# fan1994song/Sentinel

Measured on AMD Instinct MI355X. Metric: flow-check decisions/sec (node) + % HBM roofline, 10M resources, 1/2/4/8 GPU, higher is better.
Workload: dtype int64; 1 GPU; config3: 10M resources Zipf(1.1), 60% QPS / 10% THREAD / 15% WarmUp / 15% RateLimiter, acquireCount 1 (90%) or 2-5, RT~Exp(20ms) exits; events_per_batch_per_gpu=134217728, entries_per_batch_per_gpu=122837294, parallelism=resource-sharded x1, trace=config-3 batch, seed 3

## Files before the change

### sentinel_amd/csrc/sf_internal.h

```cpp
#pragma once
#include <hip/hip_runtime.h>
#include <stdint.h>

#include "../../include/sentinel_flow.h"
#include "sf_degrade.h"
#include "sf_authority.h"

namespace sf {

constexpr int64_t WS_NONE = -(1LL << 62);
constexpr int MINUTE = SF_MINUTE_BUCKETS;
constexpr int MAX_RULES = SF_MAX_RULES_PER_RESOURCE;

struct Bucket {
    int64_t ws, pass, block, exc, succ, rt, occ, min_rt;
};
struct Borrow {
    int64_t ws, pass;
};

enum : int32_t { CT_DEFAULT = 0, CT_WARM_UP = 1, CT_RATE_LIMITER = 2, CT_WARM_UP_RATE_LIMITER = 3 };

struct DevRule {
    uint8_t kind, grade;
// ... 197 lines not shown
    uint32_t arg_slots; const uint8_t* nargs; const uint8_t* atag; const uint64_t* abits;
    uint32_t arg_stride;
    const uint32_t* aoff; const uint8_t* etag; const uint64_t* ebits;
    uint32_t acsr;
    const uint32_t* origin; const uint32_t* ctx;
    int64_t base;
    const uint8_t* sys;
    const uint8_t* vprev;
    uint8_t marked;
};
struct DevVerdicts { uint8_t* status; int32_t* wait; uint16_t* rule; };

constexpr uint8_t EVF_SYSBLK = 0x80u;
constexpr uint8_t EVF_SYSREASON_SHIFT = 4;
constexpr uint8_t SYS_NONE = 0xFFu;
constexpr uint8_t SYS_INERT = 0xFEu;
constexpr uint8_t SYSR_OTHER = 7;
constexpr uint8_t SYSR_AUTH = 6;
constexpr int64_t EREF_DEAD = -2;

hipError_t query_temp_bytes(uint32_t max_n, size_t* sort_bytes, size_t* scan_bytes, size_t* pscan_bytes);
hipError_t launch_init_state(const DevState& st, hipStream_t s);
hipError_t launch_rdesc(const DevState& st, hipStream_t s);
hipError_t launch_entry_node(const DevState& st, const DevBatch& b, const uint8_t* vstatus, EntryNode* en,
                             EntryAcc* acc, hipStream_t s);
hipError_t launch_entry_init(EntryNode* en, int64_t max_rt, hipStream_t s);
hipError_t rocprim_scan_bytes(uint32_t n, size_t* bytes);
hipError_t launch_en_pack_ws(const EntryNode* en, int S, int64_t* ws, hipStream_t s);
hipError_t launch_en_pack_vals(const EntryNode* en, int S, const int64_t* gws, int64_t* vals, int64_t* minrt,
                               hipStream_t s);
hipError_t launch_snapshot(const DevState& st, int64_t now, uint32_t shard_count, uint32_t shard_index,
                           uint32_t* counts, uint32_t* offsets, sf_metric_row* out, uint32_t cap, uint32_t* total,
                           void* scan_tmp, size_t scan_bytes, hipStream_t s);
hipError_t mlog_temp_bytes(uint32_t nodes, uint32_t rows, size_t* bytes);
hipError_t launch_mlog_count(const DevState& st, EntryNode* en, bool with_entry, uint32_t shard_count,
                             uint32_t shard_index, int64_t now, unsigned long long* mask, uint32_t* counts,
                             uint32_t* offsets, uint32_t* total, void* tmp, size_t tmp_bytes, unsigned grid,
                             hipEvent_t after_count, hipStream_t s);
hipError_t launch_mlog_rows(const DevState& st, EntryNode* en, bool with_entry, uint32_t shard_count,
                            uint32_t shard_index, int64_t now, const unsigned long long* mask, const uint32_t* offsets,
                            uint32_t n_rows, sf_metric_row* rows, uint8_t* keys, uint8_t* keys_out, uint32_t* order,
                            uint32_t* order_out, void* tmp, size_t tmp_bytes, unsigned grid, hipStream_t s);
hipError_t launch_fmt_len(const sf_metric_row* rows, const uint32_t* order, uint32_t n, const char* names,
                          const uint64_t* name_off, const int32_t* types, uint32_t n_names, int64_t tz,
                          uint64_t* line_len, uint64_t* line_off, uint64_t* total, void* tmp, size_t tmp_bytes,
                          hipStream_t s);
hipError_t launch_fmt_write(const sf_metric_row* rows, const uint32_t* order, uint32_t n, const char* names,
                            const uint64_t* name_off, const int32_t* types, uint32_t n_names, int64_t tz,
                            const uint64_t* line_off, char* out, hipStream_t s);
hipError_t launch_param_stats(const DevState& st, unsigned long long* out, hipStream_t s);
size_t segs_lb_bytes(uint32_t max_n);
hipError_t launch_node_digests(const DevState& st, uint32_t n, unsigned long long* out, hipStream_t s);
hipError_t launch_param_thread_read(const DevState& st, uint32_t l, int idx, uint32_t tag, uint64_t bits,
                                    long long* out, hipStream_t s);
hipError_t launch_sort(const DevState& st, Work& w, const DevBatch& b, uint32_t shard_count, uint32_t shard_index,
                       uint32_t key_bits, hipStream_t s, hipEvent_t* ev, bool timing, bool classify = true);
struct OxWin { int64_t w0s, w0m; uint32_t ws, wm; };
struct OxPlan { uint32_t n_heavy, n_pairs; OxWin win; };
hipError_t launch_decide(const DevState& st, Work& w, const DevBatch& b, const DevVerdicts& out,
                         hipStream_t s, hipStream_t s2, hipStream_t s3, hipStream_t s4, hipEvent_t* ev, bool timing,
                         const OxPlan* ox = nullptr, bool classify = false, hipStream_t sv = nullptr);
hipError_t launch_pk_expand(const uint64_t* ev, const uint32_t* ev4, const uint32_t* ms_end, uint32_t n_ms,
                            const int64_t* xref, const int64_t* xcts, const int32_t* cext,
                            int64_t base, uint32_t n, uint32_t n_exit, uint32_t n_cext, uint2* tile_cnt,
                            uint32_t* res, int64_t* ts, int32_t* cnt, uint8_t* flags, int64_t* eref, int64_t* cts,
                            int32_t* err, hipStream_t s);
struct PkArgIn; struct PkArgOut;
struct PkCopy {
    const uint8_t* etag; const uint64_t* ebits; uint8_t* etag_out; uint64_t* ebits_out;
    const uint32_t* ctx; uint32_t* ctx_out; const uint32_t* origin; uint32_t* origin_out;
};
hipError_t launch_pk_args(const PkArgIn& in, const PkArgOut& out, const PkCopy& cp, int32_t* err, hipStream_t s);
hipError_t launch_sparse_verdicts(const int32_t* wait, const uint16_t* rule, uint32_t n, unsigned long long* wl,
                                  unsigned long long* rl, uint32_t* counts, hipStream_t s);
hipError_t launch_auth_mark(const AuthTables& t, const uint32_t* res, const uint32_t* origin, const uint8_t* flags,
                            uint32_t n, uint8_t mark, uint8_t* out, hipStream_t s);
hipError_t launch_ox_index(const DevState& st, Work& w, const DevBatch& b, uint32_t lim, hipStream_t s);
hipError_t launch_ox_apply(const DevState& st, Work& w, const DevBatch& b, uint32_t n_heavy, uint32_t n_pairs,
                           const OxWin& win, hipStream_t s);
hipError_t launch_ox_rehash(const ParamSlot* old_tab, uint64_t old_n, ParamSlot* new_tab, uint64_t new_mask,
                            int32_t* err, hipStream_t s);
hipError_t launch_aux_find(const DevState& st, uint64_t hi, uint64_t lo, uint32_t* out, hipStream_t s);
constexpr size_t ACC_BYTES = 72;
constexpr int SF_NUM_EVENTS = 18;

}
```

### sentinel_amd/csrc/sf_kernels.hip

```cpp
#include <cstring>
#include <rocprim/rocprim.hpp>

#include "sf_pkargs.h"
#include "sf_rsort.h"
#include "sf_stream.h"
#include "sf_system.h"
#include "sf_xflow.h"

namespace sf {

__global__ void k_init_state(DevState st, size_t n_sec, size_t n_min) {
    size_t i = (size_t)blockIdx.x * blockDim.x + threadIdx.x;
    size_t stride = (size_t)gridDim.x * blockDim.x;
    for (size_t k = i; k < n_sec; k += stride) {
        st.second[k] = fresh_bucket(WS_NONE, st.max_rt);
        st.borrow[k].ws = WS_NONE; st.borrow[k].pass = 0;
    }
    for (size_t k = i; k < n_min; k += stride) st.minute[k] = fresh_bucket(WS_NONE, st.max_rt);
    for (size_t k = i; k < st.R; k += stride) st.threads[k] = 0;
}

__global__ void k_segs(DevBatch b, SortedEv ev, const uint8_t* s_atag,
                       const uint32_t* keys, const uint32_t* head_scan, uint32_t* seg_start, uint32_t* seg_res,
                       uint32_t* n_seg, uint32_t* segflag, int64_t* last_ts, const int32_t* err, bool exit_marks,
// ... 1003 lines not shown
                crow.blk = (unsigned long long)v[0]; crow.succ = (unsigned long long)v[1];
                crow.rt = (unsigned long long)v[2]; crow.exc = (unsigned long long)v[3];
                crow.thr = v[4] + (long long)__popcll(__ballot(npss != 0)); crow.pass = (unsigned long long)v[5];
                crow.minrt = mr;
                crow.nblk = (unsigned)__popcll(__ballot(nblk != 0)); crow.ncmp = (unsigned)__popcll(__ballot(ncmp != 0));
                crow.nexc = (unsigned)__popcll(__ballot(nexc != 0)); crow.npass = (unsigned)__popcll(__ballot(npss != 0));
            }
            XW_PF(2)
            if (nblk || ncmp || npss) {
                if (jac) {
                    if (my_row > 0) xw_add(rows[my_row], blk, nblk, succ, rt, minrt, exc, nexc, thr, ncmp, pss, npss);
                } else if (origin != SF_ORIGIN_NONE) {
                    uint32_t h = 1 + (uint32_t)(mix64(origin) % (XW_KCAP - 1));
                    for (;;) {
                        const unsigned int prev = atomicCAS(&rows[h].key, 0u, origin + 1u);
                        if (prev == 0u || prev == origin + 1u) break;
                        h = h + 1 < XW_KCAP ? h + 1 : 1;
                    }
                    xw_add(rows[h], blk, nblk, succ, rt, minrt, exc, nexc, thr, ncmp, pss, npss);
                }
            }
            __syncthreads();
            XW_PF(3)
            if (lane == 0) xw_apply<MAXS>(cn, crow, t0);
            if constexpr (MAXS == 2) {
                if (jac) {
                    for (uint32_t k = 1 + lane; k < XW_KCAP; k += 64)
                        if ((rows[k].nblk | rows[k].ncmp | rows[k].npass | rows[k].nexc) && oc.ko[k - 1] != XNONE)
                            xw_apply<2>(xw_node(ocnw, k - 1), rows[k], t0);
                }
            }
            for (uint32_t k = 1 + lane; k < XW_KCAP && !jac; k += 64) {
                if (!rows[k].key) continue;
                const uint32_t ko = aux_get(st, l, AX_ORIGIN, rows[k].key - 1u);
                if (ko == XNONE) continue;
                NodeWin<MAXS> x;
                const NodeRows nr = aux_rows(st, ko);
                nw_load(x, st, nr);
                xw_apply<MAXS>(x, rows[k], t0);
                nw_store(x, st, nr);
            }
            XW_PF(4)
            if (act) vch[lane] = vfin;
            __syncthreads();
            jprev = j0;
            e = nx;
            XW_PF(5)
            j0 = jn;
        }
#ifdef SF_XW_PROFILE
        if (lane == 0 && hi - lo > 20000)
            printf("xw seg n=%u chunks=%llu setup=%llu solve=%llu (%llu %llu %llu %llu %llu %llu) post %llu %llu %llu %llu %llu %llu (x10ns)\n", hi - lo,
                   pf_n, pf_setup, pf_solve, pfs[0], pfs[1], pfs[2], pfs[3], pfs[4], pfs[5], pf_p[0], pf_p[1], pf_p[2], pf_p[3], pf_p[4], pf_p[5]);
#endif
        if constexpr (MAXS == 2) xw_cache_flush(st, oc, ocnw, lane);
        if (lane == 0 && cl != XNONE) nw_store(cn, st, cluster_rows(st, cl));
        __syncthreads();
    }
}

template <int MAXS>
__global__ void __launch_bounds__(128) k_decide_short_qps(DevState st, SegIO io, const uint32_t* seg_start,
                                                          const uint32_t* seg_res, LightLists ll,
                                                          const uint32_t* n_short) {
    ev_open(io.ev);
    const uint32_t t = blockIdx.x * blockDim.x + threadIdx.x;
    if (t >= n_short[1]) return;
    const uint32_t s = ll.list[ll.off[0] + ll.cap[0] - 1 - t];
    decide_qps_segment<MAXS>(st, io, seg_res[s], seg_start[s], seg_start[s + 1]);
}

static HeavyCtx heavy_ctx(const Work& w) {
    HeavyCtx hc;
    hc.seg_start = w.seg_start; hc.seg_res = w.seg_res; hc.seg_mode = w.seg_mode;
    hc.heavy_list = w.heavy_list; hc.n_heavy = w.counters + 1; hc.pcg = w.pcg; hc.seg_cap = w.seg_cap;
    hc.acc_hw = (Acc*)w.acc_hw; hc.acc_sec = (Acc*)w.acc_sec;
    hc.acc_hw_base = w.acc_hw_base; hc.acc_sec_base = w.acc_sec_base;
    hc.seg_hw0 = w.seg_hw0; hc.seg_sec0 = w.seg_sec0;
    hc.hticks = nullptr;
    hc.passbits = w.passbits;
    hc.exit_of = w.exit_of;
    hc.lxfar = w.lxfar;
    hc.thr_rec = w.thr_rec;
    hc.rid = w.keys_in; hc.run_start = w.head_scan; hc.run_pre = w.keys_out; hc.rrec = (uint2*)w.pv_in;
    hc.seg_rb = w.seg_rb; hc.seg_re = w.seg_re; hc.segflag = w.segflag;
    return hc;
}

__device__ void heavy_param(const DevState& st, const SegIO& io, const HeavyCtx& hc, uint32_t res, uint32_t lo,
                            uint32_t hi) {
    __shared__ int64_t s_now[64], s_wait[64];
    __shared__ int32_t s_c[64];
    __shared__ uint8_t s_rule[64], s_ok[64];
    const int lane = (int)(threadIdx.x & 63);
    const uint32_t p0 = st.prule_off[res], np = st.prule_off[res + 1] - p0;
    const int32_t pidx = st.prules[p0].param_idx;
    const uint8_t pm_init = (uint8_t)(st.pm_init[res] | (1u << pidx));
    ParamTable pt{st.ptab, st.pcap_mask, st.err, st.pins};
    for (uint32_t q = lo; q < hi; q += 64) {
        const uint32_t j = q + (uint32_t)lane;
        const bool valid = j < hi;
        const uint32_t jc = valid ? j : hi - 1;
        const uint32_t mw = ev_word(io, jc);
        const int64_t now = ev_time(io, mw, jc);
        const int32_t c = ev_count(io, mw, jc);
        const uint32_t na = io.arg_slots ? (io.nargs ? io.nargs[jc] : io.arg_slots) : 0;
        uint32_t tag = SF_TAG_NULL; uint64_t bits = 0;
        if ((int32_t)na > pidx) { tag = io.atag[(size_t)pidx * io.n + jc]; bits = io.abits[(size_t)pidx * io.n + jc]; }
        const bool sysb = valid && (ev_flags(mw) & EVF_SYSBLK);
        const bool key = valid && !sysb && tag != SF_TAG_NULL;
        s_now[lane] = now; s_c[lane] = c; s_wait[lane] = 0; s_rule[lane] = 0; s_ok[lane] = 0;
        unsigned long long pend = __ballot(key), mine = 0;
        while (pend) {
            const int l = __ffsll((long long)pend) - 1;
            const uint32_t kt = (uint32_t)__builtin_amdgcn_readlane((int)tag, l);
            const uint64_t kb = ((uint64_t)(uint32_t)__builtin_amdgcn_readlane((int)(uint32_t)(bits >> 32), l) << 32) |
                                (uint32_t)__builtin_amdgcn_readlane((int)(uint32_t)bits, l);
            const unsigned long long same = __ballot(key && tag == kt && bits == kb);
            if (lane == l) mine = same;
            pend &= ~same;
        }
        __syncthreads();
        if (mine) {
            uint64_t live = mine;
            for (uint32_t k = 0; k < np && live; k++) {
                const uint64_t before = live;
                live = param_run_rule(pt, res, (int)k, st.prules[p0 + k], st.items, tag, bits, live,
                                      [&](int o) { return s_now[o]; }, [&](int o) { return s_c[o]; },
                                      [&](int o, int64_t w) { s_wait[o] += w; });
                for (uint64_t m = before & ~live; m; m &= m - 1) s_rule[__builtin_ctzll(m)] = (uint8_t)k;
            }
            for (uint64_t m = live; m; m &= m - 1) s_ok[__builtin_ctzll(m)] = 1;
            if (live && ((pm_init >> pidx) & 1)) pm_thread_add(pt, res, pidx, tag, bits, __popcll(live));
        }
        __syncthreads();
        const bool blocked = sysb || (key && !s_ok[lane]);
        const unsigned long long pm = __ballot(valid && !blocked);
        if (lane == 0 && pm) {
            const uint32_t sh = q & 63;
            atomicOr(hc.passbits + (q >> 6), pm << sh);
            if (sh) atomicOr(hc.passbits + (q >> 6) + 1, pm >> (64 - sh));
        }
        if (valid) { io.v_wait[j] = (int32_t)s_wait[lane]; io.v_rule[j] = blocked && key ? s_rule[lane] : 0; }
    }
    if (lane == 0) st.pm_init[res] = pm_init;
}

template <int MAXS>
__global__ void __launch_bounds__(64) k_heavy_decide(DevState st, SegIO io, HeavyCtx hc) {
    ev_open(io.ev);
    uint32_t s;
    for (uint32_t b = blockIdx.x; heavy_at(hc, b, &s); b += gridDim.x) {
        const uint32_t lo = hc.seg_start[s], hi = hc.seg_start[s + 1], res = hc.seg_res[s];
        Team tm{(int)threadIdx.x};
        const uint64_t t_start = hc.hticks ? wall_clock64() : 0;
        switch (hc.seg_mode[s]) {
        case SM_QPS: heavy_qps<MAXS>(tm, st, io, hc, s, res, lo, hi, false); break;
        case SM_WARM: heavy_qps<MAXS>(tm, st, io, hc, s, res, lo, hi, true); break;
        case SM_NORULE: break;
        case SM_PARAM: heavy_param(st, io, hc, res, lo, hi); break;
        default:
            if (tm.leader()) decide_segment<MAXS>(st, io, res, lo, hi);
            break;
        }
        if (hc.hticks && tm.leader() && b < gridDim.x) hc.hticks[b] = wall_clock64() - t_start;
    }
}
// ... 135 lines not shown
        const uint2 tl = tiles[t];
        const uint32_t s = tl.x;
        if (hc.seg_mode[s] != SM_THREAD) { if (threadIdx.x == 0) tile_rc[t] = 0; continue; }
        if (threadIdx.x == 0) heads = 0;
        __syncthreads();
        const uint32_t lo = hc.seg_start[s], hi = hc.seg_start[s + 1];
        uint32_t nh = 0;
        bool big = false;
        for (uint32_t j = max(tl.y * FILL_TILE, lo) + threadIdx.x; j < min(tl.y * FILL_TILE + FILL_TILE, hi); j += 256) {
            const uint32_t m = ev.meta[j];
            const bool ent = is_checked_entry(ev_flags(m));
            if (ent) big |= ev_count(ev, m, j) > THR_CBIG;
            nh += (j == lo || ent != is_checked_entry(ev_flags(ev, j - 1))) ? 1u : 0u;
        }
        if (__ballot(big) && (threadIdx.x & 63) == 0) atomicOr(&segflag[s], SEGF_BIGC);
        nh = (uint32_t)wave_sum(nh);
        if ((threadIdx.x & 63) == 0 && nh) atomicAdd(&heads, nh);
        __syncthreads();
        if (threadIdx.x == 0) tile_rc[t] = heads;
        __syncthreads();
    }
}

__global__ void __launch_bounds__(1024) k_thr_rscan(uint32_t* tile_rc, const uint32_t* ntiles) {
    __shared__ uint32_t wsum[16];
    __shared__ uint32_t carry;
    const uint32_t nt = ntiles[1];
    const int lane = (int)(threadIdx.x & 63), wv = (int)(threadIdx.x >> 6);
    if (threadIdx.x == 0) carry = 0;
    __syncthreads();
    for (uint32_t b0 = 0; b0 < nt; b0 += 1024) {
        const uint32_t i = b0 + threadIdx.x;
        const uint32_t v = i < nt ? tile_rc[i] : 0u;
        const uint32_t incl = (uint32_t)wave_scan_add((int)v);
        if (lane == 63) wsum[wv] = incl;
        __syncthreads();
        uint32_t before = carry;
        for (int k = 0; k < wv; k++) before += wsum[k];
        if (i < nt) tile_rc[i] = before + incl - v;
        __syncthreads();
        if (threadIdx.x == 1023) carry = before + incl;
        __syncthreads();
    }
}

__global__ void __launch_bounds__(256) k_thr_rid(SortedEv ev, HeavyCtx hc, const uint2* tiles,
                                                 const uint32_t* ntiles, const uint32_t* tile_rb) {
    __shared__ uint32_t wsum[4];
    constexpr uint32_t PER = FILL_TILE / 256;
    const uint32_t nt = ntiles[1];
    const int lane = (int)(threadIdx.x & 63), wv = (int)(threadIdx.x >> 6);
    for (uint32_t t = blockIdx.x; t < nt; t += gridDim.x) {
        const uint2 tl = tiles[t];
        const uint32_t s = tl.x;
        if (hc.seg_mode[s] != SM_THREAD) continue;
        const uint32_t lo = hc.seg_start[s], hi = hc.seg_start[s + 1];
        const uint32_t base = tl.y * FILL_TILE + PER * threadIdx.x;
        uint32_t hm = 0;
#pragma unroll
        for (uint32_t k = 0; k < PER; k++) {
            const uint32_t j = base + k;
            if (j >= lo && j < hi && (j == lo || is_checked_entry(ev_flags(ev, j)) != is_checked_entry(ev_flags(ev, j - 1))))
                hm |= 1u << k;
        }
        const uint32_t c = (uint32_t)__popc(hm);
        const uint32_t incl = (uint32_t)wave_scan_add((int)c);
        if (lane == 63) wsum[wv] = incl;
        __syncthreads();
        uint32_t run = tile_rb[t] + incl - c;
        for (int k = 0; k < wv; k++) run += wsum[k];
        __syncthreads();
#pragma unroll
        for (uint32_t k = 0; k < PER; k++) {
            const uint32_t j = base + k;
            if (j < lo || j >= hi) continue;
            if ((hm >> k) & 1u) { run++; hc.run_start[run - 1] = j; hc.run_pre[run - 1] = 0u; }
            hc.rid[j] = run - 1;
            if (j == lo) hc.seg_rb[s] = run - 1;
            if (j == hi - 1) hc.seg_re[s] = run;
        }
    }
}

__global__ void __launch_bounds__(256) k_thr_rec(SortedEv ev, const int64_t* eref,
                                                 HeavyCtx hc, const uint2* tiles, const uint32_t* ntiles,
                                                 const uint32_t* segflag) {
    const uint32_t nt = ntiles[1];
    for (uint32_t t = blockIdx.x; t < nt; t += gridDim.x) {
        const uint2 tl = tiles[t];
        const uint32_t s = tl.x;
        if (hc.seg_mode[s] != SM_THREAD) continue;
        const uint32_t lo = hc.seg_start[s], hi = hc.seg_start[s + 1];
        const bool runs = thr_run_mode(hc, s, lo, hi, segflag[s]);
        for (uint32_t j = max(tl.y * FILL_TILE, lo) + threadIdx.x; j < min(tl.y * FILL_TILE + FILL_TILE, hi); j += 256) {
            const uint32_t m = ev.meta[j];
            const uint8_t f = ev_flags(m);
            if (runs) {
                if (is_checked_entry(f)) {
                    const uint32_t x = hc.exit_of[j];
                    hc.rrec[j] = make_uint2(x < hi ? hc.rid[x] : XO_NONE, (uint32_t)ev_count(ev, m, j));
                } else if ((f & SF_EV_EXIT) && (eref ? eref[j] : -1) == -1) {
                    atomicAdd(&hc.run_pre[hc.rid[j]], 1u);
                }
                continue;
            }
            uint2 r;
            if (is_checked_entry(f)) { r.x = hc.exit_of[j]; r.y = (uint32_t)ev_count(ev, m, j); }
            else if (!(f & SF_EV_EXIT)) { r.x = 0u; r.y = THR_REC_EXIT; }
            else {
                const int64_t ref = eref ? eref[j] : -1;
                r.x = ref >= 0 ? j - (uint32_t)ref : 0u;
                r.y = THR_REC_EXIT | (ref == -1 ? THR_REC_LIVE : 0u);
            }
            ((uint2*)hc.thr_rec)[j] = r;
        }
    }
}

constexpr int ACC_K = 32;
struct LdsAcc {
    unsigned long long v[8][ACC_K];
    long long min_rt[ACC_K];
};
__device__ __forceinline__ void lds_acc_clear(LdsAcc& A) {
    for (int i = threadIdx.x; i < 8 * ACC_K; i += blockDim.x) A.v[i / ACC_K][i % ACC_K] = 0ull;
    for (int i = threadIdx.x; i < ACC_K; i += blockDim.x) A.min_rt[i] = INT64_MAX;
}
__device__ __forceinline__ void lds_acc_add(LdsAcc& A, uint32_t k, const PAcc& p) {
    if (!p.n_touch) return;
    if (p.pass) atomicAdd(&A.v[0][k], p.pass);
    if (p.block) atomicAdd(&A.v[1][k], p.block);
    if (p.succ) atomicAdd(&A.v[2][k], p.succ);
    if (p.rt) atomicAdd(&A.v[3][k], p.rt);
    if (p.exc) atomicAdd(&A.v[4][k], p.exc);
    if (p.n_pass) atomicAdd(&A.v[5][k], p.n_pass);
    if (p.n_exit) atomicAdd(&A.v[6][k], p.n_exit);
    atomicAdd(&A.v[7][k], p.n_touch);
    if (p.min_rt != INT64_MAX) atomicMin(&A.min_rt[k], p.min_rt);
}
__device__ __forceinline__ void lds_acc_flush(LdsAcc& A, Acc* table, uint32_t base) {
    const int k = (int)threadIdx.x;
    if (k < ACC_K && A.v[7][k]) {
        PAcc p;
        p.pass = A.v[0][k]; p.block = A.v[1][k]; p.succ = A.v[2][k]; p.rt = A.v[3][k]; p.exc = A.v[4][k];
        p.n_pass = A.v[5][k]; p.n_exit = A.v[6][k]; p.n_touch = A.v[7][k]; p.min_rt = A.min_rt[k];
        p.flush(table, base + (uint32_t)k);
    }
}

constexpr int FG = (int)FILL_TILE / 256;
struct FillGrp { uint32_t m[FG]; uint8_t f[FG]; int32_t c[FG]; int64_t t[FG]; };

__device__ __forceinline__ void load16(void* dst, const void* src, int bytes) {
    if (bytes == 8) { *(uint2*)dst = *(const uint2*)src; return; }
    uint4* d = (uint4*)dst; const uint4* q = (const uint4*)src;
#pragma unroll
    for (int k = 0; k < bytes / 16; k++) d[k] = q[k];
}
__device__ __forceinline__ void store16(void* dst, const void* src, int bytes) {
    if (bytes == 8) { *(uint2*)dst = *(const uint2*)src; return; }
    uint4* d = (uint4*)dst; const uint4* q = (const uint4*)src;
#pragma unroll
    for (int k = 0; k < bytes / 16; k++) d[k] = q[k];
}

#ifndef SF_FILL_MINB
#define SF_FILL_MINB 1
#endif
__global__ void __launch_bounds__(256, SF_FILL_MINB) k_heavy_fill(DevState st, SegIO io, HeavyCtx hc, const uint2* tiles,
                                                    const uint32_t* ntiles, int cls) {
    ev_open(io.ev);
    __shared__ LdsAcc acc_h, acc_s;
    const uint32_t NONE = 0xffffffffu;
    const uint32_t nt = ntiles[cls];
    const uint32_t wl = (uint32_t)st.wl;
    const uint32_t tb = (uint32_t)((uint64_t)nt * blockIdx.x / gridDim.x);
    const uint32_t te = (uint32_t)((uint64_t)nt * (blockIdx.x + 1) / gridDim.x);
    lds_acc_clear(acc_h); lds_acc_clear(acc_s);
    uint32_t bh_k = NONE, bs_k = NONE;
    __syncthreads();
    for (uint32_t t = tb; t < te; t++) {
        const uint2 tl = tiles[t];
        const uint32_t s = tl.x;
        const uint32_t lo = hc.seg_start[s], hi = hc.seg_start[s + 1];
        const uint8_t mode = hc.seg_mode[s];
        const bool all = mode == SM_NORULE, rl = mode == SM_RL, prm = mode == SM_PARAM;
        const uint32_t hwb = hc.acc_hw_base[s], secb = hc.acc_sec_base[s];
        const int64_t hw0 = hc.seg_hw0[s], sec0 = hc.seg_sec0[s];
        const int64_t bh = hw0 * st.wl, bs = sec0 * 1000;
        const bool rel32 = ev_time(io, hi - 1) - bs < (int64_t)0xffffffffLL;
// ... 451 lines not shown
    uint32_t incl = sum;
#pragma unroll
    for (uint32_t d = 1; d < 64; d <<= 1) {
        const uint32_t y = __shfl_up(incl, d, 64);
        if (lane >= d) incl += y;
    }
    if (lane == 63u) part[wv] = incl;
    __syncthreads();
    uint32_t run = incl - sum;
    for (uint32_t q = 0; q < wv; q++) run += part[q];
    for (uint32_t q = 0; q < per; q++) {
        const uint32_t k = tid * per + q;
        if (k >= nk) break;
        const uint32_t h = hist[k];
        lbase[k] = run; run += h;
        if (h) {
            const uint32_t c = FIRST ? k : 256u + bb * nk + k;
            const uint32_t g = atomicAdd(&cursor[c], h);
            const uint64_t first = FIRST ? ((uint64_t)k << s1) : (((uint64_t)bb * nk + k) << VS_REG);
            const uint64_t cap = min((uint64_t)(FIRST ? (1ull << s1) : (1ull << VS_REG)), (uint64_t)n - min((uint64_t)n, first));
            if ((uint64_t)g + h > cap) *err = SF_ERR_INVALID;
            gbase[k] = (uint32_t)first + g - lbase[k];
        }
    }
    __syncthreads();
#pragma unroll
    for (uint32_t r = 0; r < VS_PER; r++)
        if (kr[r] != 0xffffffffu) {
            const uint32_t key = kr[r] >> 16, p = lbase[key] + (kr[r] & 0xffffu);
            buf[p] = rec[r]; kb[p] = (uint16_t)key;
        }
    __syncthreads();
    for (uint32_t k = tid; k < hi - lo; k += VS_T) {
        const uint32_t dst = gbase[kb[k]] + k;
        if (dst < n) out[dst] = buf[k];
    }
}

__global__ void __launch_bounds__(VS_T) k_vs_region(const uint32_t* in, uint8_t* o_status, uint32_t n) {
    __shared__ __align__(16) uint8_t reg[1u << VS_REG];
    const uint32_t base = blockIdx.x << VS_REG;
    const uint32_t cnt = min(1u << VS_REG, n - base);
    for (uint32_t k = threadIdx.x; k < cnt; k += VS_T) {
        const uint32_t v = in[base + k];
        reg[v & ((1u << VS_REG) - 1u)] = (uint8_t)(v >> 24);
    }
    __syncthreads();
    uint8_t* o = o_status + base;
    if (((uintptr_t)o & 15) == 0) {
        for (uint32_t k = threadIdx.x; k < cnt / 16; k += VS_T) ((uint4*)o)[k] = ((const uint4*)reg)[k];
        for (uint32_t k = (cnt & ~15u) + threadIdx.x; k < cnt; k += VS_T) o[k] = reg[k];
    } else {
        for (uint32_t k = threadIdx.x; k < cnt; k += VS_T) o[k] = reg[k];
    }
}

__global__ void k_vs_direct(const uint32_t* perm, const uint8_t* v_status, uint8_t* o_status, uint32_t n) {
    const uint32_t j = blockIdx.x * blockDim.x + threadIdx.x;
    if (j < n) o_status[perm[j]] = v_status[j];
}

static void launch_scatter(Work& w, uint32_t n, uint8_t* o_status, hipStream_t s) {
    if (n <= VS_DIRECT_MAX) {
        hipLaunchKernelGGL(k_vs_direct, dim3(blocks(n, 256)), dim3(256), 0, s, w.perm, w.v_status, o_status, n);
        return;
    }
    const uint32_t lg = 32u - (uint32_t)__builtin_clz(n - 1u);
    const uint32_t s1 = std::max(VS_REG, lg - 8u);
    const uint32_t nb1 = (uint32_t)(((uint64_t)n + (1ull << s1) - 1) >> s1);
    const uint32_t nk = 1u << (s1 - VS_REG);
    hipMemsetAsync(w.vs_cursor, 0, (256 + (size_t)nb1 * nk) * 4, s);
    hipLaunchKernelGGL(k_vs_bucket<true>, dim3((n + VS_TILE - 1) / VS_TILE), dim3(VS_T), 0, s, w.perm, w.v_status,
                       nullptr, w.keys_in, w.vs_cursor, n, s1, 0u, w.err);
    const uint32_t* regions = w.keys_in;
    if (s1 > VS_REG) {
        const uint32_t tpb = (1u << s1) / VS_TILE;
        hipLaunchKernelGGL(k_vs_bucket<false>, dim3(nb1 * tpb), dim3(VS_T), 0, s, nullptr, nullptr, w.keys_in,
                           w.keys_out, w.vs_cursor, n, s1, tpb, w.err);
        regions = w.keys_out;
    }
    hipLaunchKernelGGL(k_vs_region, dim3((n + (1u << VS_REG) - 1) >> VS_REG), dim3(VS_T), 0, s, regions, o_status, n);
}

static void launch_thr_prep(Work& w, const DevBatch& b, hipStream_t s) {
    const uint32_t n = b.n;
    HeavyCtx hc = heavy_ctx(w);
    const uint32_t tile_ub = n / FILL_TILE + n / (w.heavy_min + 1) + 2;
    const uint2* tiles1 = w.fill_tiles + w.fill_tile_cap;
    const int64_t* seref = b.eref ? w.s_eref : nullptr;
    const SortedEv ev = sorted_ev(w, b);
    const dim3 tgrid(std::min<uint32_t>(1024u, tile_ub));
    hipLaunchKernelGGL(k_thr_heads, tgrid, dim3(256), 0, s, ev, hc, tiles1, w.fill_ntiles,
                       w.tile_rc, w.segflag);
    hipLaunchKernelGGL(k_thr_rscan, dim3(1), dim3(1024), 0, s, w.tile_rc, w.fill_ntiles);
    hipLaunchKernelGGL(k_thr_rid, tgrid, dim3(256), 0, s, ev, hc, tiles1, w.fill_ntiles, w.tile_rc);
    hipLaunchKernelGGL(k_thr_rec, tgrid, dim3(256), 0, s, ev, seref, hc, tiles1, w.fill_ntiles,
                       w.segflag);
}

template <int MAXS, bool PF>
static void launch_light(const DevState& st, const SegIO& io, const Work& w, const LightLists& ll, uint32_t max_seg,
                         hipStream_t s3, hipStream_t s2) {
    const unsigned TD = 128;
    hipLaunchKernelGGL((k_decide_light<MAXS, PF>), dim3(blocks(max_seg, TD)), dim3(TD), 0, s3, st, io, w.seg_start,
                       w.seg_res, ll);
    if (st.n_window_rules) {
        hipLaunchKernelGGL(k_decide_light_qps<MAXS>, dim3(blocks(max_seg, TD)), dim3(TD), 0, s2, st, io, w.seg_start,
                           w.seg_res, ll);
        hipLaunchKernelGGL(k_decide_short_qps<MAXS>, dim3(blocks(max_seg, TD)), dim3(TD), 0, s2, st, io, w.seg_start,
                           w.seg_res, ll, w.counters + 8);
    }
    hipLaunchKernelGGL((k_decide_short<MAXS, PF>), dim3(blocks(max_seg, TD)), dim3(TD), 0, s3, st, io, w.seg_start,
                       w.seg_res, ll, w.counters + 8);
}

hipError_t launch_decide(const DevState& st, Work& w, const DevBatch& b, const DevVerdicts& out,
                         hipStream_t s, hipStream_t s2, hipStream_t s3, hipStream_t s4, hipEvent_t* ev, bool timing,
                         const OxPlan* ox, bool classify, hipStream_t sv) {
    const uint32_t n = b.n;
    if (n == 0) return hipSuccess;
    if (classify) launch_classify(st, w, b, s, ev, timing);
    SegIO io;
    io.ts = nullptr; io.cnt = nullptr; io.flags = nullptr;
    io.ev = sorted_ev(w, b);
    io.eref = b.eref ? w.s_eref : nullptr; io.cts = b.eref ? w.s_cts : nullptr;
    io.arg_slots = b.arg_slots; io.nargs = (b.arg_slots && b.nargs) ? w.s_nargs : nullptr;
    io.atag = w.s_atag; io.abits = w.s_abits; io.n = n;
    io.aoff = b.aoff; io.etag = b.etag; io.ebits = b.ebits;
    io.v_status = w.v_status; io.v_wait = w.v_wait; io.v_rule = w.v_rule;
    io.perm = w.perm; io.o_status = out.status; io.o_wait = out.wait; io.o_rule = out.rule;
    io.ev_res = b.res; io.ev_origin = b.origin; io.ev_ctx = b.ctx; io.shard_count = st.shard_count;
    HeavyCtx hc = heavy_ctx(w);
    if (timing) hc.hticks = w.hticks;
    const uint32_t max_seg = n < st.R ? n : st.R;
    const uint32_t max_heavy = n / (w.heavy_min + 1) + 1;
    StreamCtx sc{w.stream_list, w.counters + 5, w.seg_cap, timing ? w.sticks : nullptr, w.counters + 7};
    {
        FillSet f;
        if (b.eref || st.n_stream_rules) f.add(w.exit_of, (size_t)n * 4, 0xff);
        f.add(out.wait, (size_t)n * sizeof(int32_t), 0);
        f.add(out.rule, (size_t)n * sizeof(uint16_t), 0);
        launch_fill(f, s);
    }
    if (b.eref)
        hipLaunchKernelGGL(k_gather_exit, dim3(blocks(n, 256)), dim3(256), 0, s, b, w.perm, w.s_meta,
                           w.head_scan, w.seg_start, w.s_eref, w.s_cts, w.exit_of, st.err);
    hipEventRecord(ev[5], s);
    if (st.n_stream_rules) launch_thr_prep(w, b, s);
    hipEventRecord(ev[11], s);
    if (st.n_stream_rules)
        hipLaunchKernelGGL(k_heavy_stream, dim3(std::min(max_heavy, w.stream_grid)), dim3(HS_T), 0, s, st, io, hc, sc);
    hipEventRecord(ev[12], s);
    hipStreamWaitEvent(s2, ev[5], 0);
    hipStreamWaitEvent(s3, ev[5], 0);
    const bool xw_on = st.xmap && st.xw;
    auto launch_xw = [&](hipStream_t sx) {
        const unsigned g = (unsigned)std::min<size_t>((size_t)b.n / XW_MIN + 1, 2048);
        if (st.S <= 2)
            hipLaunchKernelGGL(k_decide_xw<2>, dim3(g), dim3(64), 0, sx, st, io, w.seg_start, w.seg_res,
                               w.xw_list, w.counters + 12);
        else
            hipLaunchKernelGGL(k_decide_xw<SF_MAX_SAMPLE_COUNT>, dim3(g), dim3(64), 0, sx, st, io, w.seg_start,
                               w.seg_res, w.xw_list, w.counters + 12);
        hipEventRecord(ev[15], sx);
    };
    if (xw_on) {
        hipStreamWaitEvent(s4, ev[5], 0);
        launch_xw(s4);
    }
    if (st.n_window_rules && !segs_one_pass()) {
        PcIter it(rocprim::counting_iterator<uint32_t>(0), EntryCount{sorted_ev(w, b)});
        const hipError_t e = rocprim::inclusive_scan<PcScanCfg>(w.pscan_tmp, w.pscan_tmp_bytes, it, w.pcg,
                                                                (size_t)n, rocprim::plus<int64_t>(), s2);
        if (e != hipSuccess) return e;
    }
    if (st.S <= 2)
        hipLaunchKernelGGL(k_heavy_decide<2>, dim3(max_heavy), dim3(64), 0, s2, st, io, hc);
    else
        hipLaunchKernelGGL(k_heavy_decide<SF_MAX_SAMPLE_COUNT>, dim3(max_heavy), dim3(64), 0, s2, st, io, hc);
    if (timing) hipEventRecord(ev[7], s2);
    const uint32_t fgrid = std::min<uint32_t>(w.fill_grid, n / FILL_TILE + max_heavy + 1);
    hipLaunchKernelGGL(k_heavy_fill, dim3(fgrid), dim3(256), 0, s2, st, io, hc, w.fill_tiles, w.fill_ntiles, 0);
    if (timing) hipEventRecord(ev[8], s2);
    hipLaunchKernelGGL(k_heavy_apply, dim3(blocks(max_heavy, 64)), dim3(64), 0, s2, st, hc, sc, w.seg_nhw, w.seg_nsec, 0);
    if (st.n_stream_rules) {
        hipLaunchKernelGGL(k_heavy_fill, dim3(fgrid), dim3(256), 0, s, st, io, hc,
                           w.fill_tiles + w.fill_tile_cap, w.fill_ntiles, 1);
        hipLaunchKernelGGL(k_heavy_apply, dim3(blocks(max_heavy, 64)), dim3(64), 0, s, st, hc, sc, w.seg_nhw,
                           w.seg_nsec, 1);
    }

    LightLists ll{w.light_list, w.lcounts, {}, {}};
    for (int c = 0; c < LCLS; c++) { ll.off[c] = w.loff[c]; ll.cap[c] = w.lcap[c]; }
    const bool pf = st.n_prule != 0 || st.dg_rr_of != nullptr;
    if (st.S <= 2) {
        if (pf) launch_light<2, true>(st, io, w, ll, max_seg, s3, s2);
        else launch_light<2, false>(st, io, w, ll, max_seg, s3, s2);
    } else {
        if (pf) launch_light<SF_MAX_SAMPLE_COUNT, true>(st, io, w, ll, max_seg, s3, s2);
        else launch_light<SF_MAX_SAMPLE_COUNT, false>(st, io, w, ll, max_seg, s3, s2);
    }
    if (st.xmap) {
        if (st.S <= 2)
            hipLaunchKernelGGL(k_decide_x<2>, dim3(blocks(max_seg, 64)), dim3(64), 0, s3, st, io, w.seg_start,
                               w.seg_res, w.seg_mode, w.n_seg);
        else
            hipLaunchKernelGGL(k_decide_x<SF_MAX_SAMPLE_COUNT>, dim3(blocks(max_seg, 64)), dim3(64), 0, s3, st, io,
                               w.seg_start, w.seg_res, w.seg_mode, w.n_seg);
    }
    hipEventRecord(ev[9], s3);
    hipEventRecord(ev[16], s2);
    hipEventRecord(ev[6], s2);
    hipStreamWaitEvent(s, ev[6], 0);
    hipStreamWaitEvent(s, ev[9], 0);
    hipEventRecord(ev[13], s);
    if (xw_on) hipStreamWaitEvent(s, ev[15], 0);
    if (timing) hipEventRecord(ev[3], s);
    if (ox) {
        hipStreamWaitEvent(s2, ev[13], 0);
        const hipError_t e = launch_ox_apply(st, w, b, ox->n_heavy, ox->n_pairs, ox->win, s2);
        if (e != hipSuccess) return e;
        hipEventRecord(ev[14], s2);
    }
    hipStream_t vs = sv ? sv : s;
    if (vs != s) {
        hipEventRecord(ev[17], s);
        hipStreamWaitEvent(vs, ev[17], 0);
    }
    launch_scatter(w, n, out.status, vs);
    if (ox) {
        hipStreamWaitEvent(s, ev[14], 0);
        if (vs != s) hipStreamWaitEvent(vs, ev[14], 0);
    }
// ... 227 lines not shown
```

Before: 10.08 billion decisions/s.

## Overlap thread-run table build on side stream with exit gather and fill

Splits thread-rule preparation into a table-building phase (heads, scan, run ids) launched on a secondary stream in parallel with the output fill and exit gather, and a record phase that runs after both join. The run_start buffer moves from head_scan to pv_out so the concurrent phases do not alias. The exit_of memset is dropped, and exit lookups are now validated through back-references, which avoids a full-array fill per batch. The cost is two extra events and added cross-stream synchronisation, plus the correctness risk of reading exit_of entries that were never cleared.

```diff
diff --git a/sentinel_amd/csrc/sf_internal.h b/sentinel_amd/csrc/sf_internal.h
--- a/sentinel_amd/csrc/sf_internal.h
+++ b/sentinel_amd/csrc/sf_internal.h
@@ -303,6 +303,6 @@
                             int32_t* err, hipStream_t s);
 hipError_t launch_aux_find(const DevState& st, uint64_t hi, uint64_t lo, uint32_t* out, hipStream_t s);
 constexpr size_t ACC_BYTES = 72;
-constexpr int SF_NUM_EVENTS = 18;
+constexpr int SF_NUM_EVENTS = 20;
 
 }
diff --git a/sentinel_amd/csrc/sf_kernels.hip b/sentinel_amd/csrc/sf_kernels.hip
--- a/sentinel_amd/csrc/sf_kernels.hip
+++ b/sentinel_amd/csrc/sf_kernels.hip
@@ -1109,7 +1109,7 @@
     hc.exit_of = w.exit_of;
     hc.lxfar = w.lxfar;
     hc.thr_rec = w.thr_rec;
-    hc.rid = w.keys_in; hc.run_start = w.head_scan; hc.run_pre = w.keys_out; hc.rrec = (uint2*)w.pv_in;
+    hc.rid = w.keys_in; hc.run_start = (uint32_t*)w.pv_out; hc.run_pre = w.keys_out; hc.rrec = (uint2*)w.pv_in;
     hc.seg_rb = w.seg_rb; hc.seg_re = w.seg_re; hc.segflag = w.segflag;
     return hc;
 }
@@ -1411,6 +1411,17 @@
     }
 }
 
+__device__ __forceinline__ uint32_t thr_exit_of(const SortedEv& ev, const int64_t* eref, const HeavyCtx& hc,
+                                                uint32_t j, uint32_t hi, const uint32_t* of) {
+    if (!eref) return XO_NONE;
+    const uint32_t x = hc.exit_of[j];
+    if (x <= j || x >= hi) return XO_NONE;
+    const uint8_t fx = ev_flags(ev, x);
+    const int64_t back = eref[x];
+    const uint32_t v = of ? of[x] : x;
+    return ((fx & SF_EV_EXIT) && back == (int64_t)j) ? v : XO_NONE;
+}
+
 __global__ void __launch_bounds__(256) k_thr_rec(SortedEv ev, const int64_t* eref,
                                                  HeavyCtx hc, const uint2* tiles, const uint32_t* ntiles,
                                                  const uint32_t* segflag) {
@@ -1426,15 +1437,14 @@
             const uint8_t f = ev_flags(m);
             if (runs) {
                 if (is_checked_entry(f)) {
-                    const uint32_t x = hc.exit_of[j];
-                    hc.rrec[j] = make_uint2(x < hi ? hc.rid[x] : XO_NONE, (uint32_t)ev_count(ev, m, j));
+                    hc.rrec[j] = make_uint2(thr_exit_of(ev, eref, hc, j, hi, hc.rid), (uint32_t)ev_count(ev, m, j));
                 } else if ((f & SF_EV_EXIT) && (eref ? eref[j] : -1) == -1) {
                     atomicAdd(&hc.run_pre[hc.rid[j]], 1u);
                 }
                 continue;
             }
             uint2 r;
-            if (is_checked_entry(f)) { r.x = hc.exit_of[j]; r.y = (uint32_t)ev_count(ev, m, j); }
+            if (is_checked_entry(f)) { r.x = thr_exit_of(ev, eref, hc, j, hi, nullptr); r.y = (uint32_t)ev_count(ev, m, j); }
             else if (!(f & SF_EV_EXIT)) { r.x = 0u; r.y = THR_REC_EXIT; }
             else {
                 const int64_t ref = eref ? eref[j] : -1;
@@ -2052,20 +2062,25 @@
     hipLaunchKernelGGL(k_vs_region, dim3((n + (1u << VS_REG) - 1) >> VS_REG), dim3(VS_T), 0, s, regions, o_status, n);
 }
 
-static void launch_thr_prep(Work& w, const DevBatch& b, hipStream_t s) {
-    const uint32_t n = b.n;
+static dim3 thr_prep_grid(const Work& w, uint32_t n) {
+    return dim3(std::min<uint32_t>(1024u, n / FILL_TILE + n / (w.heavy_min + 1) + 2));
+}
+static void launch_thr_tables(Work& w, const DevBatch& b, hipStream_t s) {
     HeavyCtx hc = heavy_ctx(w);
-    const uint32_t tile_ub = n / FILL_TILE + n / (w.heavy_min + 1) + 2;
     const uint2* tiles1 = w.fill_tiles + w.fill_tile_cap;
-    const int64_t* seref = b.eref ? w.s_eref : nullptr;
     const SortedEv ev = sorted_ev(w, b);
-    const dim3 tgrid(std::min<uint32_t>(1024u, tile_ub));
+    const dim3 tgrid = thr_prep_grid(w, b.n);
     hipLaunchKernelGGL(k_thr_heads, tgrid, dim3(256), 0, s, ev, hc, tiles1, w.fill_ntiles,
                        w.tile_rc, w.segflag);
     hipLaunchKernelGGL(k_thr_rscan, dim3(1), dim3(1024), 0, s, w.tile_rc, w.fill_ntiles);
     hipLaunchKernelGGL(k_thr_rid, tgrid, dim3(256), 0, s, ev, hc, tiles1, w.fill_ntiles, w.tile_rc);
-    hipLaunchKernelGGL(k_thr_rec, tgrid, dim3(256), 0, s, ev, seref, hc, tiles1, w.fill_ntiles,
-                       w.segflag);
+}
+static void launch_thr_rec(Work& w, const DevBatch& b, hipStream_t s) {
+    HeavyCtx hc = heavy_ctx(w);
+    const uint2* tiles1 = w.fill_tiles + w.fill_tile_cap;
+    const int64_t* seref = b.eref ? w.s_eref : nullptr;
+    hipLaunchKernelGGL(k_thr_rec, thr_prep_grid(w, b.n), dim3(256), 0, s, sorted_ev(w, b), seref, hc, tiles1,
+                       w.fill_ntiles, w.segflag);
 }
 
 template <int MAXS, bool PF>
@@ -2105,9 +2120,14 @@
     const uint32_t max_seg = n < st.R ? n : st.R;
     const uint32_t max_heavy = n / (w.heavy_min + 1) + 1;
     StreamCtx sc{w.stream_list, w.counters + 5, w.seg_cap, timing ? w.sticks : nullptr, w.counters + 7};
+    const bool thr = st.n_stream_rules != 0;
+    if (thr) {
+        if (s2 != s) { hipEventRecord(ev[18], s); hipStreamWaitEvent(s2, ev[18], 0); }
+        launch_thr_tables(w, b, s2);
+        if (s2 != s) hipEventRecord(ev[19], s2);
+    }
     {
         FillSet f;
-        if (b.eref || st.n_stream_rules) f.add(w.exit_of, (size_t)n * 4, 0xff);
         f.add(out.wait, (size_t)n * sizeof(int32_t), 0);
         f.add(out.rule, (size_t)n * sizeof(uint16_t), 0);
         launch_fill(f, s);
@@ -2115,10 +2135,11 @@
     if (b.eref)
         hipLaunchKernelGGL(k_gather_exit, dim3(blocks(n, 256)), dim3(256), 0, s, b, w.perm, w.s_meta,
                            w.head_scan, w.seg_start, w.s_eref, w.s_cts, w.exit_of, st.err);
+    if (thr && s2 != s) hipStreamWaitEvent(s, ev[19], 0);
+    if (thr) launch_thr_rec(w, b, s);
     hipEventRecord(ev[5], s);
-    if (st.n_stream_rules) launch_thr_prep(w, b, s);
     hipEventRecord(ev[11], s);
-    if (st.n_stream_rules)
+    if (thr)
         hipLaunchKernelGGL(k_heavy_stream, dim3(std::min(max_heavy, w.stream_grid)), dim3(HS_T), 0, s, st, io, hc, sc);
     hipEventRecord(ev[12], s);
     hipStreamWaitEvent(s2, ev[5], 0);
```

New measurement: 10.05 billion decisions/s. Within noise of the previous version (-0.2%).
